# Quantum-Chemistry-Group-BNU/XTDDFT

Measured on NVIDIA B200. Metric: davidson_sigma_vectors_per_s, higher is better.
Workload: dtype f64

## Files before the change

### xtddft_b200/csrc/ozaki.cuh

```cuda
#pragma once
#include "common.cuh"

namespace xtd {

constexpr int OZ_BM = 128, OZ_BN = 64, OZ_KB = 32, OZ_STAGES = 4, OZ_MAX_S = 8, OZ_MIN_S = 3;
constexpr int OZ_THREADS = 192;
constexpr int OZ_K1_THREADS = 320;

__device__ __forceinline__ uint32_t oz_smem_u32(const void* p) { return (uint32_t)__cvta_generic_to_shared(p); }

__device__ __forceinline__ double oz_scale_of(double m) {
  if (!(m > 1e-280 && m < 1e280)) return 0.0;
  int e;
  frexp(m, &e);
  return ldexp(1.0, e - 6);
}

__global__ void oz_rowmax_t_kernel(double* __restrict__ scale, int rows_pad, const double* __restrict__ X, long ld, long sq, int rows, int K,
                                   int nq, int group, long k_valid) {
  const int row = blockIdx.x * 32 + threadIdx.x, g = blockIdx.y;
  double m = 0.0;
  if (row < rows) {
    const int q1 = min(nq, (g + 1) * group);
    for (int q = g * group; q < q1; ++q) {
      const long kmax = min((long)K, k_valid - (long)q * K);
      const double* x = X + (long)q * sq + row;
      for (long k = threadIdx.y; k < kmax; k += 32) m = fmax(m, fabs(x[k * ld]));
    }
  }
  __shared__ double red[32][33];
  red[threadIdx.y][threadIdx.x] = m;
  __syncthreads();
  if (threadIdx.y == 0) {
    for (int w = 1; w < 32; ++w) m = fmax(m, red[w][threadIdx.x]);
    if (row < rows_pad) scale[(long)g * rows_pad + row] = oz_scale_of(m);
  }
}

__global__ void oz_rowmax_kernel(double* __restrict__ scale, int rows_pad, const double* __restrict__ X, long ld, long sq, int rows, int K,
                                 int nq, int group, long k_valid) {
  const int row = blockIdx.x, g = blockIdx.y;
  double m = 0.0;
  if (row < rows) {
    const int q1 = min(nq, (g + 1) * group);
    for (int q = g * group; q < q1; ++q) {
      const int kmax = (int)min((long)K, k_valid - (long)q * K);
      const double* x = X + (long)q * sq + (long)row * ld;
      for (int k = threadIdx.x; k < kmax; k += blockDim.x) m = fmax(m, fabs(x[k]));
    }
  }
  __shared__ double red[8];
  for (int o = 16; o > 0; o >>= 1) m = fmax(m, __shfl_xor_sync(0xffffffffu, m, o));
  if ((threadIdx.x & 31) == 0) red[threadIdx.x >> 5] = m;
  __syncthreads();
  if (threadIdx.x == 0) {
    for (int w = 1; w < (int)(blockDim.x >> 5); ++w) m = fmax(m, red[w]);
    scale[(long)g * rows_pad + row] = oz_scale_of(m);
  }
}

template <int S>
__device__ __forceinline__ void oz_digits16(const double (&t)[16], uint32_t (&pk)[S][4]) {
  const double magic = 6755399441055744.0;
  if constexpr (S <= 6) {
    constexpr double SCL = (double)(1ull << (8 * (S - 1)));
    constexpr unsigned long long BAL = 128ull * (((1ull << (8 * (S - 1))) - 1ull) / 255ull);
    constexpr unsigned long long CADD = BAL - 0x4338000000000000ull;
#pragma unroll
    for (int w = 0; w < 4; ++w) {
      uint32_t lo[4], hi[4];
#pragma unroll
      for (int j = 0; j < 4; ++j) {
// ... 22 lines not shown
      for (int sl = 0; sl < S; ++sl) {
        const double u = (sl == 0) ? __dadd_rd(tt, magic) : __fma_rd(tt, 256.0, magic);
        const double qd = u - magic;
        tt = (sl == 0) ? (tt - qd) : fma(tt, 256.0, -qd);
        dg[sl] = __double2loint(u);
      }
      int carry = 0;
#pragma unroll
      for (int sl = S - 1; sl >= 1; --sl) {
        const int vv = dg[sl] + carry;
        carry = vv >= 128 ? 1 : 0;
        dg[sl] = vv - (carry << 8);
      }
      dg[0] += carry;
#pragma unroll
      for (int sl = 0; sl < S; ++sl) pk[sl][k >> 2] |= ((uint32_t)dg[sl] & 0xffu) << ((k & 3) * 8);
    }
  }
}

template <int S, bool TRANS>
__global__ void __launch_bounds__(128) oz_slice_kernel(int8_t* __restrict__ out, const double* __restrict__ scale, int rows_pad,
                                                       const double* __restrict__ X, long ld, long sq, int rows, int K, int RT, int nkb,
                                                       int group, int stacked, long k_valid) {
  const int c2 = blockIdx.x, q = blockIdx.z;
  const int row = blockIdx.y * 128 + threadIdx.x;
  const int rt = row / RT, r = row - rt * RT, nrt = rows_pad / RT;
  const int k0 = c2 * 16;
  double x[16];
#pragma unroll
  for (int k = 0; k < 16; ++k) x[k] = 0.0;
  double sc = 0.0;
  if (row < rows) {
    sc = scale[(long)(q / group) * rows_pad + row];
    const int kmax = (int)min((long)K, k_valid - (long)q * K);
    if (TRANS) {
      const double* src = X + (long)q * sq + (long)k0 * ld + row;
#pragma unroll
      for (int k = 0; k < 16; ++k)
        if (k0 + k < kmax) x[k] = src[(long)k * ld];
    } else {
      const double* src = X + (long)q * sq + (long)row * ld + k0;
      if (k0 + 16 <= kmax) {
#pragma unroll
        for (int k = 0; k < 16; k += 2) {
          const double2 v = *reinterpret_cast<const double2*>(src + k);
          x[k] = v.x;
          x[k + 1] = v.y;
        }
      } else {
#pragma unroll
        for (int k = 0; k < 16; ++k)
          if (k0 + k < kmax) x[k] = src[k];
      }
    }
  }
  const double inv = sc > 0.0 ? __hiloint2double(0x7fe00000 - __double2hiint(sc), 0) : 0.0;
  uint32_t pk[S][4];
#pragma unroll
  for (int k = 0; k < 16; ++k) x[k] *= inv;
  oz_digits16<S>(x, pk);
  int8_t* dst = out + ((((long)q * nrt + rt) * nkb + (c2 >> 1)) * S) * ((long)RT * OZ_KB) + (long)r * 16 +
                (stacked ? (long)(c2 & 1) * S * RT * 16 : (long)(c2 & 1) * RT * 16);
  const long plane = stacked ? (long)RT * 16 : (long)RT * OZ_KB;
#pragma unroll
// ... 364 lines not shown
#pragma unroll
        for (int k = 0; k < HC; ++k) acc[k] = fma(v[k], sa * sb[k], acc[k]);
      }
      double* w = p.W + zb * p.w_bstride + ((long)sp * p.Mpad + mt * OZ_BM + row) * p.Npad + nt * OZ_BN + half * HC;
#pragma unroll
      for (int c = 0; c < HC; c += 2) *reinterpret_cast<double2*>(w + c) = make_double2(p.alpha * acc[c], p.alpha * acc[c + 1]);
    }
  }
  asm volatile("tcgen05.fence::before_thread_sync;" ::: "memory");
  __syncthreads();
  if (warp == 1) {
    asm volatile("tcgen05.fence::after_thread_sync;" ::: "memory");
    asm volatile("tcgen05.dealloc.cta_group::1.sync.aligned.b32 %0, %1;" ::"r"(tmem_base), "r"(512u) : "memory");
  }
}

struct OzK1Params {
  const int8_t* A;
  const int8_t* B;
  const double* sa;
  const double* sb;
  const double* so;
  int8_t* out;
  int np, nit, nbt, nkb1, nvec, no, group, nmt2, nkb2, Mpad2;
  int it0, nit_run;
  int i_lo, i_hi;
  long ntiles;
};

template <int S>
__global__ void __launch_bounds__(OZ_K1_THREADS, 1) oz_k1_kernel(const OzK1Params p) {
  constexpr int A_SLICE = OZ_BM * OZ_KB, B_SLICE = OZ_BN * OZ_KB;
  constexpr int A_BYTES = S * A_SLICE, B_BYTES = S * B_SLICE, STAGE = A_BYTES + B_BYTES;
  extern __shared__ __align__(128) uint8_t oz_smem[];
  uint64_t* full = reinterpret_cast<uint64_t*>(oz_smem + OZ_STAGES * STAGE);
  uint64_t* empty = full + OZ_STAGES;
  uint64_t* tmem_full = empty + OZ_STAGES;
  uint64_t* tmem_empty = tmem_full + 1;
  uint32_t* tmem_slot = reinterpret_cast<uint32_t*>(tmem_empty + 1);
  const int warp = threadIdx.x >> 5, lane = threadIdx.x & 31;

  if (threadIdx.x == 0) {
    for (int s = 0; s < OZ_STAGES; ++s) {
      oz_mbar_init(&full[s], 1);
      oz_mbar_init(&empty[s], 1);
    }
    oz_mbar_init(tmem_full, 1);
    oz_mbar_init(tmem_empty, OZ_K1_THREADS - 64);
    asm volatile("fence.mbarrier_init.release.cluster;" ::: "memory");
    asm volatile("fence.proxy.async.shared::cta;" ::: "memory");
  }
  if (warp == 1) {
    asm volatile("tcgen05.alloc.cta_group::1.sync.aligned.shared::cta.b32 [%0], %1;" ::"r"(oz_smem_u32(tmem_slot)), "r"(512u) : "memory");
    asm volatile("tcgen05.relinquish_alloc_permit.cta_group::1.sync.aligned;" ::: "memory");
  }
  asm volatile("tcgen05.fence::before_thread_sync;" ::: "memory");
  __syncthreads();
  asm volatile("tcgen05.fence::after_thread_sync;" ::: "memory");
  const uint32_t tmem_base = *tmem_slot;
  const long per_p = (long)p.nit_run * p.nvec * p.nbt, per_it = (long)p.nvec * p.nbt;

  if (warp == 0) {
    if (lane == 0) {
      long it = 0;
      for (long t = blockIdx.x; t < p.ntiles; t += gridDim.x) {
        const int P = (int)(t / per_p);
        const long r0 = t - (long)P * per_p;
        const int itile = (int)(r0 / per_it);
        const long r1 = r0 - (long)itile * per_it;
        const int x = (int)(r1 / p.nbt), bt = (int)(r1 - (long)x * p.nbt);
        const int8_t* a = p.A + (((long)P * p.nit + p.it0 + itile) * p.nkb1) * A_BYTES;
        const int8_t* b = p.B + (((long)x * p.nbt + bt) * p.nkb1) * B_BYTES;
        for (int kb = 0; kb < p.nkb1; ++kb, ++it) {
          const int s = (int)(it % OZ_STAGES);
          const uint32_t ph = (uint32_t)((it / OZ_STAGES) & 1);
          oz_mbar_wait(&empty[s], ph ^ 1u);
          oz_mbar_expect_tx(&full[s], STAGE);
          uint8_t* sa = oz_smem + s * STAGE;
          oz_bulk_load(sa, a + (long)kb * A_BYTES, A_BYTES, &full[s]);
          oz_bulk_load(sa + A_BYTES, b + (long)kb * B_BYTES, B_BYTES, &full[s]);
        }
      }
    }
  } else if (warp == 1) {
    if (lane == 0) {
      constexpr uint32_t idesc0 = (2u << 4) | (1u << 7) | (1u << 10) | ((uint32_t)(OZ_BM >> 4) << 24);
      const uint32_t smem_base = oz_smem_u32(oz_smem);
      long it = 0, n = 0;
      for (long t = blockIdx.x; t < p.ntiles; t += gridDim.x, ++n) {
        if (n > 0) oz_mbar_wait(tmem_empty, (uint32_t)((n - 1) & 1));
        asm volatile("tcgen05.fence::after_thread_sync;" ::: "memory");
        for (int kb = 0; kb < p.nkb1; ++kb, ++it) {
          const int s = (int)(it % OZ_STAGES);
          const uint32_t ph = (uint32_t)((it / OZ_STAGES) & 1);
          oz_mbar_wait(&full[s], ph);
          asm volatile("tcgen05.fence::after_thread_sync;" ::: "memory");
          const uint32_t a_base = smem_base + s * STAGE, b_base = a_base + A_BYTES;
          const uint32_t later = kb > 0 ? 1u : 0u;
#pragma unroll
          for (int i = 0; i < S; ++i) {
            const uint64_t da = oz_smem_desc(a_base + i * A_SLICE, OZ_BM * 16, 128);
#pragma unroll
            for (int j0 = 0; j0 < S - i; j0 += 4) {
              const int nj = (S - i - j0) < 4 ? (S - i - j0) : 4;
              const uint64_t db = oz_smem_desc(b_base + j0 * (OZ_BN * 16), S * OZ_BN * 16, 128);
              const uint32_t idesc = idesc0 | ((uint32_t)((nj * OZ_BN) >> 3) << 17);
              oz_mma_i8(tmem_base + (uint32_t)((i + j0) * OZ_BN), da, db, idesc, (i > 0) ? 1u : later);
            }
          }
          oz_commit(&empty[s]);
        }
        oz_commit(tmem_full);
      }
    }
  } else {
    const int quad = warp & 3, half = (warp - 2) >> 2;
    const int row = quad * 32 + lane;
    const uint32_t taddr = tmem_base + ((uint32_t)(quad * 32) << 16);
    const double magic = 6755399441055744.0;
    const int rowsA = p.nit * OZ_BM, rowsB = p.nbt * OZ_BN;
    long n = 0;
    for (long t = blockIdx.x; t < p.ntiles; t += gridDim.x, ++n) {
      const int P = (int)(t / per_p);
      const long r0 = t - (long)P * per_p;
      const int itile = p.it0 + (int)(r0 / per_it);
      const long r1 = r0 - (long)(itile - p.it0) * per_it;
      const int x = (int)(r1 / p.nbt), bt = (int)(r1 - (long)x * p.nbt);
      const int i = itile * OZ_BM + row;
      const bool valid = i >= p.i_lo && i < p.i_hi;
      const int m = x * p.no + i;
      const double sa = valid ? p.sa[(long)P * rowsA + i] : 0.0;
      const double so = valid ? p.so[(long)(P / p.group) * p.Mpad2 + m] : 0.0;
      const double inv = so > 0.0 ? __hiloint2double(0x7fe00000 - __double2hiint(so), 0) : 0.0;
      const double f = sa * inv;
      const double* sb = p.sb + (long)x * rowsB + bt * OZ_BN;
      int8_t* dst = p.out + ((((long)P * p.nmt2 + (m >> 7)) * p.nkb2 + bt * 2) * S) * (long)A_SLICE + (long)(m & 127) * 16;
      oz_mbar_wait(tmem_full, (uint32_t)(n & 1));
      asm volatile("tcgen05.fence::after_thread_sync;" ::: "memory");
      constexpr int HC = OZ_BN / 2;
      double v[HC];
#pragma unroll
      for (int k = 0; k < HC; ++k) v[k] = 0.0;
#pragma unroll
      for (int l = S - 1; l >= 0; --l) {
        uint32_t r[HC];
#pragma unroll
        for (int cc = 0; cc < HC; cc += 16) oz_tmem_ld16(taddr + (uint32_t)(l * OZ_BN + half * HC + cc), r + cc);
        asm volatile("tcgen05.wait::ld.sync.aligned;" ::: "memory");
#pragma unroll
        for (int k = 0; k < HC; ++k)
          v[k] = fma(v[k], 0.00390625, __hiloint2double(0x43300000, (int)(r[k] ^ 0x80000000u)) - 4503601774854144.0);
      }
      asm volatile("tcgen05.fence::before_thread_sync;" ::: "memory");
      oz_mbar_arrive(tmem_empty);
#pragma unroll
      for (int cc = 0; cc < HC; cc += 16) {
        const int c0 = half * HC + cc;
        uint32_t pk[S][4];
        double tt[16];
#pragma unroll
        for (int k = 0; k < 16; ++k) tt[k] = v[cc + k] * (f * sb[c0 + k]);
        oz_digits16<S>(tt, pk);
        if (valid && bt * 2 + (c0 >> 5) < p.nkb2) {
          int8_t* d = dst + (long)(c0 >> 5) * S * A_SLICE + ((c0 >> 4) & 1) * (OZ_BM * 16);
#pragma unroll
          for (int sl = 0; sl < S; ++sl) *reinterpret_cast<uint4*>(d + (long)sl * A_SLICE) = make_uint4(pk[sl][0], pk[sl][1], pk[sl][2], pk[sl][3]);
        }
      }
    }
  }
  asm volatile("tcgen05.fence::before_thread_sync;" ::: "memory");
  __syncthreads();
  if (warp == 1) {
    asm volatile("tcgen05.fence::after_thread_sync;" ::: "memory");
    asm volatile("tcgen05.dealloc.cta_group::1.sync.aligned.b32 %0, %1;" ::"r"(tmem_base), "r"(512u) : "memory");
  }
}

__global__ void oz_rownorm_kernel(double* __restrict__ out, int rows_pad, const double* __restrict__ X, long ld, long sq, int rows, int K) {
  const int row = blockIdx.x, q = blockIdx.y;
  double a = 0.0;
  if (row < rows) {
    const double* x = X + (long)q * sq + (long)row * ld;
    for (int k = threadIdx.x; k < K; k += blockDim.x) a = fma(x[k], x[k], a);
  }
  __shared__ double red[8];
  for (int o = 16; o > 0; o >>= 1) a += __shfl_xor_sync(0xffffffffu, a, o);
  if ((threadIdx.x & 31) == 0) red[threadIdx.x >> 5] = a;
  __syncthreads();
  if (threadIdx.x == 0) {
    for (int w = 1; w < (int)(blockDim.x >> 5); ++w) a += red[w];
    out[(long)q * rows_pad + row] = sqrt(a);
  }
}
__global__ void oz_colmax_kernel(double* __restrict__ zmax, const double* __restrict__ norms, int rows_pad, int rows) {
// ... 7 lines not shown
  if (threadIdx.x == 0) {
    for (int w = 1; w < (int)(blockDim.x >> 5); ++w) m = fmax(m, red[w]);
    zmax[x] = m;
  }
}
__global__ void oz_bound_scale_kernel(double* __restrict__ so, int Mpad2, const double* __restrict__ loo_norm, int rowsA, const double* __restrict__ zmax,
                                      int np, int group, int nvec, int no, int i_lo, int i_hi) {
  const int m = blockIdx.x * blockDim.x + threadIdx.x, g = blockIdx.y;
  if (m >= Mpad2) return;
  double s = 0.0;
  if (m < nvec * no) {
    const int x = m / no, i = m - x * no;
    if (i < i_lo || i >= i_hi) return;
    double nl = 0.0;
    const int p1 = min(np, (g + 1) * group);
    for (int P = g * group; P < p1; ++P) nl = fmax(nl, loo_norm[(long)P * rowsA + i]);
    s = oz_scale_of(nl * zmax[x] * (1.0 + 1e-9));
  } else if (i_lo != 0) {
    return;
  }
  so[(long)g * Mpad2 + m] = s;
}

template <int S>
inline int oz_k1_launch(const OzK1Params& p, int num_sms, cudaStream_t st) {
  static bool attr_set[64] = {false};
  int dev = 0;
  XTD_CUDA(cudaGetDevice(&dev));
  if (!attr_set[dev & 63]) {
    XTD_CUDA(cudaFuncSetAttribute(oz_k1_kernel<S>, cudaFuncAttributeMaxDynamicSharedMemorySize, (int)((size_t)OZ_STAGES * S * (OZ_BM + OZ_BN) * OZ_KB + 256)));
    attr_set[dev & 63] = true;
  }
  const unsigned grid = (unsigned)std::min<long>(p.ntiles, num_sms);
  oz_k1_kernel<S><<<grid, OZ_K1_THREADS, (size_t)OZ_STAGES * S * (OZ_BM + OZ_BN) * OZ_KB + 256, st>>>(p);
  XTD_COUNT_LAUNCH();
  XTD_CUDA(cudaGetLastError());
  return XTD_OK;
}

inline int oz_k1(int S, const OzK1Params& p, int num_sms, cudaStream_t st) {
  switch (S) {
    case 3: return oz_k1_launch<3>(p, num_sms, st);
    case 4: return oz_k1_launch<4>(p, num_sms, st);
    case 5: return oz_k1_launch<5>(p, num_sms, st);
    case 6: return oz_k1_launch<6>(p, num_sms, st);
    case 7: return oz_k1_launch<7>(p, num_sms, st);
    case 8: return oz_k1_launch<8>(p, num_sms, st);
  }
  XTD_SET_ERR("oz_k1: %d slices (3..8)", S);
  return XTD_ERR_ARG;
}

struct OzShape {
  int rows = 0, RT = 0, rows_pad = 0, nrt = 0, K = 0, nkb = 0;
  void set(int rows_, int RT_, int K_) {
    rows = rows_; RT = RT_; K = K_;
    rows_pad = (int)round_up(rows_, 128);
    nrt = rows_pad / RT_;
    nkb = (int)cdiv(K_, OZ_KB);
  }
  size_t slice_bytes(long nq, int S) const { return (size_t)nq * nrt * nkb * S * RT * OZ_KB; }
  size_t scale_doubles(long nq, int group) const { return (size_t)cdiv(nq, group) * rows_pad; }
};

inline size_t oz_gemm_smem(int S) { return (size_t)OZ_STAGES * S * (OZ_BM + OZ_BN) * OZ_KB + 256; }

inline int oz_max_group(int K, int S) {
  const long kpad = round_up(K, OZ_KB);
  const long g = ((1L << 31) - 1) / ((long)S * 16384 * kpad);
  return (int)std::max<long>(g, 0);
}

template <int S>
inline int oz_slice_launch(int8_t* out, double* scale, const OzShape& sh, const double* X, long ld, long sq, int nq, int group,
                           bool trans, long k_valid, cudaStream_t st) {
  const int ng = (int)cdiv(nq, group);
  const int stacked = sh.RT == OZ_BN ? 1 : 0;
  const dim3 sgrid(2 * sh.nkb, sh.rows_pad / 128, nq);
  if (trans) {
    oz_rowmax_t_kernel<<<dim3(sh.rows_pad / 32, ng), dim3(32, 32), 0, st>>>(scale, sh.rows_pad, X, ld, sq, sh.rows, sh.K, nq, group, k_valid);
    XTD_COUNT_LAUNCH();
    XTD_CUDA(cudaGetLastError());
    oz_slice_kernel<S, true><<<sgrid, 128, 0, st>>>(out, scale, sh.rows_pad, X, ld, sq, sh.rows, sh.K, sh.RT, sh.nkb, group, stacked, k_valid);
  } else {
    oz_rowmax_kernel<<<dim3(sh.rows_pad, ng), 256, 0, st>>>(scale, sh.rows_pad, X, ld, sq, sh.rows, sh.K, nq, group, k_valid);
    XTD_COUNT_LAUNCH();
    XTD_CUDA(cudaGetLastError());
    oz_slice_kernel<S, false><<<sgrid, 128, 0, st>>>(out, scale, sh.rows_pad, X, ld, sq, sh.rows, sh.K, sh.RT, sh.nkb, group, stacked, k_valid);
  }
  XTD_COUNT_LAUNCH();
  XTD_CUDA(cudaGetLastError());
  return XTD_OK;
}

inline int oz_slice(int S, int8_t* out, double* scale, const OzShape& sh, const double* X, long ld, long sq, int nq, int group,
                    cudaStream_t st, bool trans = false, long k_valid = 0) {
  XTD_REQUIRE(nq >= 1 && nq <= 65535, XTD_ERR_ARG, "oz_slice: %d q-slices per launch (1..65535)", nq);
  XTD_REQUIRE(trans || (ld % 2 == 0 && sq % 2 == 0 && ((uintptr_t)X & 15) == 0), XTD_ERR_ALIGN,
              "oz_slice: operand must be 16-byte aligned with even strides");
  if (k_valid <= 0) k_valid = (long)nq * sh.K;
  switch (S) {
    case 3: return oz_slice_launch<3>(out, scale, sh, X, ld, sq, nq, group, trans, k_valid, st);
    case 4: return oz_slice_launch<4>(out, scale, sh, X, ld, sq, nq, group, trans, k_valid, st);
    case 5: return oz_slice_launch<5>(out, scale, sh, X, ld, sq, nq, group, trans, k_valid, st);
    case 6: return oz_slice_launch<6>(out, scale, sh, X, ld, sq, nq, group, trans, k_valid, st);
    case 7: return oz_slice_launch<7>(out, scale, sh, X, ld, sq, nq, group, trans, k_valid, st);
    case 8: return oz_slice_launch<8>(out, scale, sh, X, ld, sq, nq, group, trans, k_valid, st);
  }
  XTD_SET_ERR("oz_slice: %d slices (3..8)", S);
  return XTD_ERR_ARG;
}

template <int S, int CN>
inline int oz_gemm_launch_cn(const OzGemmParams& p, cudaStream_t st) {
  static bool attr_set[64] = {false};
  int dev = 0;
  XTD_CUDA(cudaGetDevice(&dev));
  if (!attr_set[dev & 63]) {
    XTD_CUDA(cudaFuncSetAttribute(oz_gemm_kernel<S, CN>, cudaFuncAttributeMaxDynamicSharedMemorySize, (int)oz_gemm_smem(S)));
    attr_set[dev & 63] = true;
  }
  cudaLaunchConfig_t cfg = {};
  cfg.gridDim = dim3((unsigned)(p.nmt * p.nnt * p.splits), (unsigned)p.batches);
  cfg.blockDim = dim3(OZ_THREADS);
  cfg.dynamicSmemBytes = oz_gemm_smem(S);
  cfg.stream = st;
  cudaLaunchAttribute attr[1];
  attr[0].id = cudaLaunchAttributeClusterDimension;
  attr[0].val.clusterDim.x = CN;
  attr[0].val.clusterDim.y = 1;
// ... 70 lines not shown
```

### xtddft_b200/csrc/xtd_api.cu

```cuda
#include "../../include/xtd_sigma.h"
#include "gemm.cuh"
#include "kernels.cuh"
#include "ozaki.cuh"
#include "davidson.cuh"

#include <cuda_profiler_api.h>

#include <algorithm>
#include <cstring>
#include <vector>

namespace xtd {
thread_local char g_last_error[512] = {0};
unsigned long long g_launch_count = 0;

struct DevBuf {
  double* p = nullptr;
  size_t bytes = 0;
  DevBuf() = default;
  DevBuf(const DevBuf&) = delete;
  DevBuf& operator=(const DevBuf&) = delete;
  ~DevBuf() { release(); }
  int alloc(size_t n_doubles, cudaStream_t s) {
    release();
// ... 15 lines not shown
  std::vector<std::pair<int, int>> o_blocks, v_blocks;
  long ldz, ldzt, ldco, ldcv, ldN;
  DevBuf Co, Cv, CoT, CvT;
  DevBuf Loo[2], Lvv[2];
  DevBuf Loob[2][2];
  bool need_split[2] = {false, false};
  DevBuf Lvo[2];
  bool need_narrow[2] = {false, false};
  DevBuf Lvt[2];
  DevBuf Lov[2];
  bool need_kt[2] = {false, false};
  int tail_start = 0, tail_w = 0;
  long ldoo, ldvv;
  bool need_k[2] = {false, false};
  bool use_oz[2] = {false, false};
  int8_t* LvvS[2] = {nullptr, nullptr};
  double* LvvScale[2] = {nullptr, nullptr};
  OzShape ozB;
  int oz_group = 0;
  int oz_col0[2] = {0, 0};
  int8_t* LooS[2] = {nullptr, nullptr};
  double *LooScale[2] = {nullptr, nullptr}, *LooNorm[2] = {nullptr, nullptr};
  OzShape ozL;
  bool xc_oz = false;
  int8_t *phivF = nullptr, *phivB = nullptr;
  double *phivFs = nullptr, *phivBs = nullptr;
  OzShape ozPF, ozPB;
  bool xc_oz_split = false;
  int8_t *phiF = nullptr, *phiB = nullptr;
  double *phiFs = nullptr, *phiBs = nullptr;
  OzShape ozOF, ozOB;
  DevBuf phi;
  long ldphi = 0;
  DevBuf phiv;
  long ldphiv = 0;
  long *g_indptr = nullptr, *g_cols = nullptr;
  double* g_vals = nullptr;
  long g_nnz = 0;
};

constexpr long XC_SPLIT_SMEM_MAX = 200 * 1024;
constexpr int XC_OP_MAX_NVEC = 8;
constexpr int OZ_XC_KQ = 8192;
constexpr int NARROW_MAX = 16;

struct KTermRec {
// ... 593 lines not shown
    XTD_TRY(c->Loo[tensor].alloc((size_t)naux_local * c->no * c->ldoo, h->stream));
    c->use_oz[tensor] = false;
    c->oz_col0[tensor] = 0;
    if (h->oz_slices > 0 && oz_max_group(c->nv, h->oz_slices) >= 1) {
      int n_uni = 0, n_blk = 0;
      for (const KTermRec& k : h->kterms)
        if (k.tensor == tensor && h->ch[k.ch] == c) (k.uniform ? n_uni : n_blk)++;
      if (n_blk == 0) c->use_oz[tensor] = n_uni > 0;
      else if (n_uni == 0) {
        if (c->v_blocks.size() == 1) c->use_oz[tensor] = true;
        else if (c->need_narrow[tensor]) { c->use_oz[tensor] = true; c->oz_col0[tensor] = c->v_blocks[1].first; }
      }
      if (c->use_oz[tensor]) c->tail_w = 0;
    }
    if (c->use_oz[tensor]) {
      c->ozB.set(c->nv - c->oz_col0[tensor], OZ_BN, c->nv);
      c->oz_group = std::min(4, oz_max_group(c->nv, h->oz_slices));
      if (c->LvvS[tensor]) cudaFree(c->LvvS[tensor]);
      if (c->LvvScale[tensor]) cudaFree(c->LvvScale[tensor]);
      c->LvvS[tensor] = nullptr; c->LvvScale[tensor] = nullptr;
      XTD_CUDA(cudaMalloc((void**)&c->LvvS[tensor], std::max<size_t>(c->ozB.slice_bytes(naux_local, h->oz_slices), 16)));
      XTD_CUDA(cudaMalloc((void**)&c->LvvScale[tensor], std::max<size_t>(c->ozB.scale_doubles(naux_local, c->oz_group), 2) * 8));
      c->Lvv[tensor].release();
      c->ozL.set(c->no, OZ_BM, c->no);
      if (c->LooS[tensor]) cudaFree(c->LooS[tensor]);
      if (c->LooScale[tensor]) cudaFree(c->LooScale[tensor]);
      if (c->LooNorm[tensor]) cudaFree(c->LooNorm[tensor]);
      c->LooS[tensor] = nullptr; c->LooScale[tensor] = c->LooNorm[tensor] = nullptr;
      XTD_CUDA(cudaMalloc((void**)&c->LooS[tensor], std::max<size_t>(c->ozL.slice_bytes(naux_local, h->oz_slices), 16)));
      XTD_CUDA(cudaMalloc((void**)&c->LooScale[tensor], std::max<size_t>((size_t)naux_local * c->ozL.rows_pad, 2) * 8));
      XTD_CUDA(cudaMalloc((void**)&c->LooNorm[tensor], std::max<size_t>((size_t)naux_local * c->ozL.rows_pad, 2) * 8));
    } else {
      XTD_TRY(c->Lvv[tensor].alloc((size_t)naux_local * c->nv * c->ldvv, h->stream));
    }
    if (c->need_narrow[tensor]) XTD_TRY(c->Lvo[tensor].alloc((size_t)naux_local * c->v_blocks[1].first * c->ldvv, h->stream));
    if (c->need_narrow[tensor] && c->tail_w > 0) XTD_TRY(c->Lvt[tensor].alloc((size_t)naux_local * c->tail_w * c->ldvv, h->stream));
    if (c->need_split[tensor]) {
      const int o2 = c->o_blocks[1].first;
      XTD_TRY(c->Loob[tensor][0].alloc((size_t)naux_local * o2 * c->ldoo, h->stream));
      XTD_TRY(c->Loob[tensor][1].alloc((size_t)naux_local * (c->no - o2) * c->ldoo, h->stream));
    }
  }
  if (tensor == 0)
    for (auto* j : h->jblocks) XTD_TRY(j->L.alloc((size_t)naux_local * j->nr * j->ld, h->stream));
  return XTD_OK;
}

int xtd_df_add(xtd_handle h, int tensor, const double* l_dev, long np, long ld_row, long stride_p, int packed) {
  XTD_REQUIRE(h && (tensor == 0 || tensor == 1) && l_dev && np > 0, XTD_ERR_ARG, "xtd_df_add: bad arguments");
  XTD_REQUIRE(h->naux_filled[tensor] + np <= h->naux[tensor], XTD_ERR_ARG, "xtd_df_add: more aux rows than declared (%ld + %ld > %ld)",
              h->naux_filled[tensor], np, h->naux[tensor]);
  const int N = h->nao;
  const long ldN = h->ldN;
  cudaStream_t s = h->stream;
// ... 73 lines not shown
      f.M = nmo; f.N = nmo; f.K = pn * nu_;
      f.C = h->kopen.p; f.ldc = h->ld_mo; f.accumulate = true;
      XTD_TRY(gemm(h->gemm, f, s));
    }
    for (size_t ci = 0; ci < h->ch.size(); ++ci) {
      Channel* c = h->ch[ci];
      bool need_o = c->need_k[tensor] || c->need_kt[tensor];
      if (tensor == 0)
        for (auto* j : h->jblocks) need_o = need_o || (j->ch == (int)ci);
      if (need_o) {
        GemmDesc d;
        d.A = view2d(c->CoT.p, ldN, c->no, N); d.B = Lv; d.M = c->no; d.N = N; d.K = N;
        d.batches = pn; d.z_div = 1; d.a_hi = 0; d.b_hi = 1;
        d.C = half; d.ldc = ldN; d.c_batch_stride = (long)c->no * ldN;
        XTD_TRY(gemm(h->gemm, d, s));
        MatView Hv = view3d(half, ldN, (long)c->no * ldN, pn, c->no, N);
        if (c->need_k[tensor]) {
          GemmDesc e;
          e.A = Hv; e.B = view2d(c->CoT.p, ldN, c->no, N); e.M = c->no; e.N = c->no; e.K = N;
          e.batches = pn; e.a_hi = 1; e.b_hi = 0;
          e.C = c->Loo[tensor].p + P0 * c->no * c->ldoo; e.ldc = c->ldoo; e.c_batch_stride = (long)c->no * c->ldoo;
          XTD_TRY(gemm(h->gemm, e, s));
          if (c->use_oz[tensor]) {
            const double* lc = c->Loo[tensor].p + P0 * c->no * c->ldoo;
            XTD_TRY(oz_slice(h->oz_slices, c->LooS[tensor] + c->ozL.slice_bytes(P0, h->oz_slices), c->LooScale[tensor] + (size_t)P0 * c->ozL.rows_pad,
                             c->ozL, lc, c->ldoo, (long)c->no * c->ldoo, pn, 1, s));
            oz_rownorm_kernel<<<dim3(c->ozL.rows_pad, pn), 128, 0, s>>>(c->LooNorm[tensor] + (size_t)P0 * c->ozL.rows_pad, c->ozL.rows_pad, lc, c->ldoo,
                                                                        (long)c->no * c->ldoo, c->no, c->no);
            LAUNCH_CHECK();
          }
          if (c->need_split[tensor]) {
            const int o2 = c->o_blocks[1].first;
            const int r0s[2] = {0, o2}, nrs[2] = {o2, c->no - o2};
            for (int ib = 0; ib < 2; ++ib) {
              GemmDesc f = e;
              f.A = view3d(half, ldN, (long)c->no * ldN, pn, nrs[ib], N, r0s[ib], 0);
              f.M = nrs[ib];
              f.C = c->Loob[tensor][ib].p + P0 * nrs[ib] * c->ldoo; f.c_batch_stride = (long)nrs[ib] * c->ldoo;
              XTD_TRY(gemm(h->gemm, f, s));
            }
          }
        }
        if (c->need_kt[tensor]) {
          GemmDesc e;
          e.A = Hv; e.B = view2d(c->CvT.p, ldN, c->nv, N);
          e.M = c->no; e.N = c->nv; e.K = N; e.batches = pn; e.a_hi = 1; e.b_hi = 0;
          e.C = c->Lov[tensor].p + P0 * c->no * c->ldz; e.ldc = c->ldz; e.c_batch_stride = (long)c->no * c->ldz;
          XTD_TRY(gemm(h->gemm, e, s));
        }
        if (tensor == 0)
          for (auto* j : h->jblocks) {
// ... 739 lines not shown
    PhaseTimer t(h, XTD_T_K2_SLICE);
    for (int ip = 0; ip < npass; ++ip) {
      const double* zt = h->ZT[k.ch];
      if (!k.uniform) {
        scale_blocks_kernel<<<dim3((unsigned)cdiv(ch->no, 128), ch->nv, nvec), 128, 0, s>>>(zts_tmp, h->ZT[k.ch], ch->ldzt, (long)ch->nv * ch->ldzt,
                                                                                          ch->nv, ch->no, passes[ip].bs);
        LAUNCH_CHECK();
        zt = zts_tmp;
      }
      XTD_TRY(oz_slice(S, ztS[ip], ztScale[ip], shZt, zt, ch->ldzt, (long)ch->nv * ch->ldzt, nvec, 1, s));
      oz_rownorm_kernel<<<dim3(shZt.rows_pad, nvec), 128, 0, s>>>(ztNorm, shZt.rows_pad, zt, ch->ldzt, (long)ch->nv * ch->ldzt, ch->nv, ch->no);
      LAUNCH_CHECK();
      oz_colmax_kernel<<<nvec, 256, 0, s>>>(zmax[ip], ztNorm, shZt.rows_pad, ch->nv);
      LAUNCH_CHECK();
    }
  }
  for (long P0 = 0; P0 < naux; P0 += pc) {
    const int pn = (int)std::min<long>(pc, naux - P0);
    const int ng = (int)cdiv(pn, G);
    {
      PhaseTimer t(h, XTD_T_K1);
      for (int ip = 0; ip < npass; ++ip) {
        const RowPass& rp = passes[ip];
        oz_bound_scale_kernel<<<dim3((unsigned)cdiv(shA.rows_pad, 256), ng), 256, 0, s>>>(so, shA.rows_pad, ch->LooNorm[k.tensor] + (size_t)P0 * shL.rows_pad,
                                                                                          shL.rows_pad, zmax[ip], pn, G, nvec, ch->no, rp.i_lo, rp.i_hi);
        LAUNCH_CHECK();
        OzK1Params q;
        q.A = ch->LooS[k.tensor] + shL.slice_bytes(P0, S); q.B = ztS[ip];
        q.sa = ch->LooScale[k.tensor] + (size_t)P0 * shL.rows_pad; q.sb = ztScale[ip]; q.so = so; q.out = As;
        q.np = pn; q.nit = shL.nrt; q.nbt = shZt.nrt; q.nkb1 = shL.nkb; q.nvec = nvec; q.no = ch->no; q.group = G;
        q.nmt2 = shA.nrt; q.nkb2 = shA.nkb; q.Mpad2 = shA.rows_pad;
        q.i_lo = rp.i_lo; q.i_hi = rp.i_hi;
        q.it0 = rp.i_lo / OZ_BM; q.nit_run = (rp.i_hi - 1) / OZ_BM - q.it0 + 1;
        q.ntiles = (long)pn * q.nit_run * nvec * q.nbt;
        XTD_TRY(oz_k1(S, q, h->gemm.num_sms, s));
        h->gemm.flops += 2.0 * pn * (double)(rp.i_hi - rp.i_lo) * ch->no * ch->nv * nvec;
      }
    }
    {
      PhaseTimer t(h, XTD_T_K2);
      OzGemmParams p;
      p.A = As; p.B = ch->LvvS[k.tensor]; p.sa = so; p.sb = ch->LvvScale[k.tensor];
      p.nmt = shA.nrt; p.nnt = shB.nrt; p.nkb = shA.nkb; p.nq = pn; p.group = G; p.b_q0 = (int)P0;
      p.Mpad = shA.rows_pad; p.Npad = shB.rows_pad;
      p.splits = std::min(splits_max, oz_choose_splits(tiles, ng, h->gemm.num_sms));
      p.W = W; p.alpha = k.uniform ? k.w[0][0][0][0] : 1.0;
      XTD_TRY(oz_gemm(S, p, s));
      const int M = nvec * ch->no, N = ch->nv - col0;
      const long nblk = cdiv((long)M * N, 256);
      reduce_splits_kernel<<<dim3((unsigned)(nblk > 4096 ? 4096 : nblk), 1), 256, 0, s>>>(
          h->SIG + h->sig_base[k.ch] + col0, ch->ldz, 0, W, shB.rows_pad, 0, (long)shA.rows_pad * shB.rows_pad, p.splits, M, N, 1, 0, 0, 0);
      LAUNCH_CHECK();
      h->gemm.flops += 2.0 * M * N * (double)ch->nv * pn;
    }
  }
  return XTD_OK;
}

// ... 903 lines not shown
```

Baseline: 9.482.

## Pack Loo rows across aux groups and multicast A tiles in 2-CTA clusters

Loo slices are now packed so that G auxiliary indices share one row dimension, with rows split at the occupied-block boundary. This fills the 128-row M tiles instead of padding a small `no` to 128 per P. The K1 fused kernel now runs as 2-CTA clusters where each CTA loads half of the shared A tile and multicasts it to both, while each processes a different B tile. Empty-buffer barriers count two arrivals and commits are multicast, which adds cluster synchronization and index unpacking overhead in the epilogue. Warps whose rows are all invalid skip the store path.

```diff
diff --git a/xtddft_b200/csrc/ozaki.cuh b/xtddft_b200/csrc/ozaki.cuh
--- a/xtddft_b200/csrc/ozaki.cuh
+++ b/xtddft_b200/csrc/ozaki.cuh
@@ -8,6 +8,32 @@
 constexpr int OZ_K1_THREADS = 320;
 
 __device__ __forceinline__ uint32_t oz_smem_u32(const void* p) { return (uint32_t)__cvta_generic_to_shared(p); }
+
+__host__ __device__ __forceinline__ bool oz_unpack_row(int r, int G, int o2, int no, int& P, int& i) {
+  if (r < G * o2) {
+    P = r / o2;
+    i = r - P * o2;
+    return true;
+  }
+  const int n1 = no - o2, r1 = r - G * o2;
+  if (r1 >= G * n1) return false;
+  P = r1 / n1;
+  i = o2 + (r1 - P * n1);
+  return true;
+}
+inline int oz_packed_row_lo(int i_lo, int G, int o2) { return i_lo >= o2 ? G * o2 : 0; }
+inline int oz_packed_row_hi(int i_hi, int G, int o2, int no) { return i_hi <= o2 ? G * o2 : G * no; }
+
+struct OzRowPack {
+  int G = 0, o2 = 0, no = 0, np = 0;
+  long sp = 0;
+};
+__device__ __forceinline__ long oz_src_row(const OzRowPack& pk, int q, int row, int rows, long ld) {
+  if (pk.G == 0) return row < rows ? (long)row * ld : -1L;
+  int P, i;
+  if (!oz_unpack_row(row, pk.G, pk.o2, pk.no, P, i) || q * pk.G + P >= pk.np) return -1L;
+  return (long)P * pk.sp + (long)i * ld;
+}
 
 __device__ __forceinline__ double oz_scale_of(double m) {
   if (!(m > 1e-280 && m < 1e280)) return 0.0;
@@ -38,16 +64,16 @@
 }
 
 __global__ void oz_rowmax_kernel(double* __restrict__ scale, int rows_pad, const double* __restrict__ X, long ld, long sq, int rows, int K,
-                                 int nq, int group, long k_valid) {
+                                 int nq, int group, long k_valid, const OzRowPack pack) {
   const int row = blockIdx.x, g = blockIdx.y;
   double m = 0.0;
-  if (row < rows) {
-    const int q1 = min(nq, (g + 1) * group);
-    for (int q = g * group; q < q1; ++q) {
-      const int kmax = (int)min((long)K, k_valid - (long)q * K);
-      const double* x = X + (long)q * sq + (long)row * ld;
-      for (int k = threadIdx.x; k < kmax; k += blockDim.x) m = fmax(m, fabs(x[k]));
-    }
+  const int q1 = min(nq, (g + 1) * group);
+  for (int q = g * group; q < q1; ++q) {
+    const long off = oz_src_row(pack, q, row, rows, ld);
+    if (off < 0) continue;
+    const int kmax = (int)min((long)K, k_valid - (long)q * K);
+    const double* x = X + (long)q * sq + off;
+    for (int k = threadIdx.x; k < kmax; k += blockDim.x) m = fmax(m, fabs(x[k]));
   }
   __shared__ double red[8];
   for (int o = 16; o > 0; o >>= 1) m = fmax(m, __shfl_xor_sync(0xffffffffu, m, o));
@@ -116,7 +142,7 @@
 template <int S, bool TRANS>
 __global__ void __launch_bounds__(128) oz_slice_kernel(int8_t* __restrict__ out, const double* __restrict__ scale, int rows_pad,
                                                        const double* __restrict__ X, long ld, long sq, int rows, int K, int RT, int nkb,
-                                                       int group, int stacked, long k_valid) {
+                                                       int group, int stacked, long k_valid, const OzRowPack pack) {
   const int c2 = blockIdx.x, q = blockIdx.z;
   const int row = blockIdx.y * 128 + threadIdx.x;
   const int rt = row / RT, r = row - rt * RT, nrt = rows_pad / RT;
@@ -125,7 +151,8 @@
 #pragma unroll
   for (int k = 0; k < 16; ++k) x[k] = 0.0;
   double sc = 0.0;
-  if (row < rows) {
+  const long off = TRANS ? (row < rows ? 0L : -1L) : oz_src_row(pack, q, row, rows, ld);
+  if (off >= 0) {
     sc = scale[(long)(q / group) * rows_pad + row];
     const int kmax = (int)min((long)K, k_valid - (long)q * K);
     if (TRANS) {
@@ -134,7 +161,7 @@
       for (int k = 0; k < 16; ++k)
         if (k0 + k < kmax) x[k] = src[(long)k * ld];
     } else {
-      const double* src = X + (long)q * sq + (long)row * ld + k0;
+      const double* src = X + (long)q * sq + off + k0;
       if (k0 + 16 <= kmax) {
 #pragma unroll
         for (int k = 0; k < 16; k += 2) {
@@ -545,16 +572,37 @@
   const double* sb;
   const double* so;
   int8_t* out;
-  int np, nit, nbt, nkb1, nvec, no, group, nmt2, nkb2, Mpad2;
-  int it0, nit_run;
+  int np, ntg, nbt, nkb1, nvec, no, o2, group, nmt2, nkb2, Mpad2;
+  int t0, nt_run;
   int i_lo, i_hi;
-  long ntiles;
+  long npairs;
 };
+
+struct OzK1Item {
+  int gl, tile, x, bt;
+  bool live;
+};
+__device__ __forceinline__ OzK1Item oz_k1_item(const OzK1Params& p, long u, uint32_t crank) {
+  const long nxb = (long)p.nvec * p.nbt, nxb2 = (nxb + 1) >> 1, per_g = (long)p.nt_run * nxb2;
+  OzK1Item t;
+  t.gl = (int)(u / per_g);
+  const long r0 = u - (long)t.gl * per_g;
+  const int itile = (int)(r0 / nxb2);
+  t.tile = p.t0 + itile;
+  long xb = 2 * (r0 - (long)itile * nxb2) + crank;
+  t.live = xb < nxb;
+  if (!t.live) xb = nxb - 1;
+  t.x = (int)(xb / p.nbt);
+  t.bt = (int)(xb - (long)t.x * p.nbt);
+  return t;
+}
 
 template <int S>
 __global__ void __launch_bounds__(OZ_K1_THREADS, 1) oz_k1_kernel(const OzK1Params p) {
   constexpr int A_SLICE = OZ_BM * OZ_KB, B_SLICE = OZ_BN * OZ_KB;
   constexpr int A_BYTES = S * A_SLICE, B_BYTES = S * B_SLICE, STAGE = A_BYTES + B_BYTES;
+  constexpr int A_HALF = A_BYTES / 2;
+  constexpr uint16_t cmask = 3;
   extern __shared__ __align__(128) uint8_t oz_smem[];
   uint64_t* full = reinterpret_cast<uint64_t*>(oz_smem + OZ_STAGES * STAGE);
   uint64_t* empty = full + OZ_STAGES;
@@ -562,11 +610,13 @@
   uint64_t* tmem_empty = tmem_full + 1;
   uint32_t* tmem_slot = reinterpret_cast<uint32_t*>(tmem_empty + 1);
   const int warp = threadIdx.x >> 5, lane = threadIdx.x & 31;
+  const uint32_t crank = oz_cluster_rank();
+  const long pair0 = blockIdx.x >> 1, npair_ctas = gridDim.x >> 1;
 
   if (threadIdx.x == 0) {
     for (int s = 0; s < OZ_STAGES; ++s) {
       oz_mbar_init(&full[s], 1);
-      oz_mbar_init(&empty[s], 1);
+      oz_mbar_init(&empty[s], 2);
     }
     oz_mbar_init(tmem_full, 1);
     oz_mbar_init(tmem_empty, OZ_K1_THREADS - 64);
@@ -579,28 +629,24 @@
   }
   asm volatile("tcgen05.fence::before_thread_sync;" ::: "memory");
   __syncthreads();
+  oz_cluster_sync();
   asm volatile("tcgen05.fence::after_thread_sync;" ::: "memory");
   const uint32_t tmem_base = *tmem_slot;
-  const long per_p = (long)p.nit_run * p.nvec * p.nbt, per_it = (long)p.nvec * p.nbt;
 
   if (warp == 0) {
     if (lane == 0) {
       long it = 0;
-      for (long t = blockIdx.x; t < p.ntiles; t += gridDim.x) {
-        const int P = (int)(t / per_p);
-        const long r0 = t - (long)P * per_p;
-        const int itile = (int)(r0 / per_it);
-        const long r1 = r0 - (long)itile * per_it;
-        const int x = (int)(r1 / p.nbt), bt = (int)(r1 - (long)x * p.nbt);
-        const int8_t* a = p.A + (((long)P * p.nit + p.it0 + itile) * p.nkb1) * A_BYTES;
-        const int8_t* b = p.B + (((long)x * p.nbt + bt) * p.nkb1) * B_BYTES;
+      for (long u = pair0; u < p.npairs; u += npair_ctas) {
+        const OzK1Item t = oz_k1_item(p, u, crank);
+        const int8_t* a = p.A + (((long)t.gl * p.ntg + t.tile) * p.nkb1) * A_BYTES + crank * A_HALF;
+        const int8_t* b = p.B + (((long)t.x * p.nbt + t.bt) * p.nkb1) * B_BYTES;
         for (int kb = 0; kb < p.nkb1; ++kb, ++it) {
           const int s = (int)(it % OZ_STAGES);
           const uint32_t ph = (uint32_t)((it / OZ_STAGES) & 1);
           oz_mbar_wait(&empty[s], ph ^ 1u);
           oz_mbar_expect_tx(&full[s], STAGE);
           uint8_t* sa = oz_smem + s * STAGE;
-          oz_bulk_load(sa, a + (long)kb * A_BYTES, A_BYTES, &full[s]);
+          oz_bulk_load_mc(sa + crank * A_HALF, a + (long)kb * A_BYTES, A_HALF, &full[s], cmask);
           oz_bulk_load(sa + A_BYTES, b + (long)kb * B_BYTES, B_BYTES, &full[s]);
         }
       }
@@ -610,7 +656,7 @@
       constexpr uint32_t idesc0 = (2u << 4) | (1u << 7) | (1u << 10) | ((uint32_t)(OZ_BM >> 4) << 24);
       const uint32_t smem_base = oz_smem_u32(oz_smem);
       long it = 0, n = 0;
-      for (long t = blockIdx.x; t < p.ntiles; t += gridDim.x, ++n) {
+      for (long u = pair0; u < p.npairs; u += npair_ctas, ++n) {
         if (n > 0) oz_mbar_wait(tmem_empty, (uint32_t)((n - 1) & 1));
         asm volatile("tcgen05.fence::after_thread_sync;" ::: "memory");
         for (int kb = 0; kb < p.nkb1; ++kb, ++it) {
@@ -631,7 +677,7 @@
               oz_mma_i8(tmem_base + (uint32_t)((i + j0) * OZ_BN), da, db, idesc, (i > 0) ? 1u : later);
             }
           }
-          oz_commit(&empty[s]);
+          oz_commit_mc(&empty[s], cmask);
         }
         oz_commit(tmem_full);
       }
@@ -640,20 +686,18 @@
     const int quad = warp & 3, half = (warp - 2) >> 2;
     const int row = quad * 32 + lane;
     const uint32_t taddr = tmem_base + ((uint32_t)(quad * 32) << 16);
-    const double magic = 6755399441055744.0;
-    const int rowsA = p.nit * OZ_BM, rowsB = p.nbt * OZ_BN;
+    const int rowsA = p.ntg * OZ_BM, rowsB = p.nbt * OZ_BN;
     long n = 0;
-    for (long t = blockIdx.x; t < p.ntiles; t += gridDim.x, ++n) {
-      const int P = (int)(t / per_p);
-      const long r0 = t - (long)P * per_p;
-      const int itile = p.it0 + (int)(r0 / per_it);
-      const long r1 = r0 - (long)(itile - p.it0) * per_it;
-      const int x = (int)(r1 / p.nbt), bt = (int)(r1 - (long)x * p.nbt);
-      const int i = itile * OZ_BM + row;
-      const bool valid = i >= p.i_lo && i < p.i_hi;
+    for (long u = pair0; u < p.npairs; u += npair_ctas, ++n) {
+      const OzK1Item t = oz_k1_item(p, u, crank);
+      const int x = t.x, bt = t.bt;
+      const int pr = t.tile * OZ_BM + row;
+      int Pl = 0, i = 0;
+      const bool valid = t.live && oz_unpack_row(pr, p.group, p.o2, p.no, Pl, i) && i >= p.i_lo && i < p.i_hi && t.gl * p.group + Pl < p.np;
+      const int P = t.gl * p.group + Pl;
       const int m = x * p.no + i;
-      const double sa = valid ? p.sa[(long)P * rowsA + i] : 0.0;
-      const double so = valid ? p.so[(long)(P / p.group) * p.Mpad2 + m] : 0.0;
+      const double sa = valid ? p.sa[(long)t.gl * rowsA + pr] : 0.0;
+      const double so = valid ? p.so[(long)t.gl * p.Mpad2 + m] : 0.0;
       const double inv = so > 0.0 ? __hiloint2double(0x7fe00000 - __double2hiint(so), 0) : 0.0;
       const double f = sa * inv;
       const double* sb = p.sb + (long)x * rowsB + bt * OZ_BN;
@@ -676,6 +720,7 @@
       }
       asm volatile("tcgen05.fence::before_thread_sync;" ::: "memory");
       oz_mbar_arrive(tmem_empty);
+      if (!__any_sync(0xffffffffu, valid)) continue;
 #pragma unroll
       for (int cc = 0; cc < HC; cc += 16) {
         const int c0 = half * HC + cc;
@@ -694,6 +739,7 @@
   }
   asm volatile("tcgen05.fence::before_thread_sync;" ::: "memory");
   __syncthreads();
+  oz_cluster_sync();
   if (warp == 1) {
     asm volatile("tcgen05.fence::after_thread_sync;" ::: "memory");
     asm volatile("tcgen05.dealloc.cta_group::1.sync.aligned.b32 %0, %1;" ::"r"(tmem_base), "r"(512u) : "memory");
@@ -747,30 +793,47 @@
   so[(long)g * Mpad2 + m] = s;
 }
 
+inline size_t oz_gemm_smem(int S) { return (size_t)OZ_STAGES * S * (OZ_BM + OZ_BN) * OZ_KB + 256; }
+
 template <int S>
-inline int oz_k1_launch(const OzK1Params& p, int num_sms, cudaStream_t st) {
+inline int oz_k1_launch(const OzK1Params& p, cudaStream_t st) {
   static bool attr_set[64] = {false};
+  static int max_clusters[64] = {0};
   int dev = 0;
   XTD_CUDA(cudaGetDevice(&dev));
+  cudaLaunchConfig_t cfg = {};
+  cfg.blockDim = dim3(OZ_K1_THREADS);
+  cfg.dynamicSmemBytes = oz_gemm_smem(S);
+  cfg.stream = st;
+  cudaLaunchAttribute attr[1];
+  attr[0].id = cudaLaunchAttributeClusterDimension;
+  attr[0].val.clusterDim.x = 2;
+  attr[0].val.clusterDim.y = 1;
+  attr[0].val.clusterDim.z = 1;
+  cfg.attrs = attr;
+  cfg.numAttrs = 1;
   if (!attr_set[dev & 63]) {
-    XTD_CUDA(cudaFuncSetAttribute(oz_k1_kernel<S>, cudaFuncAttributeMaxDynamicSharedMemorySize, (int)((size_t)OZ_STAGES * S * (OZ_BM + OZ_BN) * OZ_KB + 256)));
+    XTD_CUDA(cudaFuncSetAttribute(oz_k1_kernel<S>, cudaFuncAttributeMaxDynamicSharedMemorySize, (int)oz_gemm_smem(S)));
+    cfg.gridDim = dim3(2);
+    XTD_CUDA(cudaOccupancyMaxActiveClusters(&max_clusters[dev & 63], oz_k1_kernel<S>, &cfg));
+    XTD_REQUIRE(max_clusters[dev & 63] >= 1, XTD_ERR_CUDA, "oz_k1: no 2-CTA cluster of the fused half-transform fits this device");
     attr_set[dev & 63] = true;
   }
-  const unsigned grid = (unsigned)std::min<long>(p.ntiles, num_sms);
-  oz_k1_kernel<S><<<grid, OZ_K1_THREADS, (size_t)OZ_STAGES * S * (OZ_BM + OZ_BN) * OZ_KB + 256, st>>>(p);
+  cfg.gridDim = dim3((unsigned)(2 * std::min<long>(p.npairs, max_clusters[dev & 63])));
+  XTD_CUDA(cudaLaunchKernelEx(&cfg, oz_k1_kernel<S>, p));
   XTD_COUNT_LAUNCH();
   XTD_CUDA(cudaGetLastError());
   return XTD_OK;
 }
 
-inline int oz_k1(int S, const OzK1Params& p, int num_sms, cudaStream_t st) {
+inline int oz_k1(int S, const OzK1Params& p, cudaStream_t st) {
   switch (S) {
-    case 3: return oz_k1_launch<3>(p, num_sms, st);
-    case 4: return oz_k1_launch<4>(p, num_sms, st);
-    case 5: return oz_k1_launch<5>(p, num_sms, st);
-    case 6: return oz_k1_launch<6>(p, num_sms, st);
-    case 7: return oz_k1_launch<7>(p, num_sms, st);
-    case 8: return oz_k1_launch<8>(p, num_sms, st);
+    case 3: return oz_k1_launch<3>(p, st);
+    case 4: return oz_k1_launch<4>(p, st);
+    case 5: return oz_k1_launch<5>(p, st);
+    case 6: return oz_k1_launch<6>(p, st);
+    case 7: return oz_k1_launch<7>(p, st);
+    case 8: return oz_k1_launch<8>(p, st);
   }
   XTD_SET_ERR("oz_k1: %d slices (3..8)", S);
   return XTD_ERR_ARG;
@@ -788,8 +851,6 @@
   size_t scale_doubles(long nq, int group) const { return (size_t)cdiv(nq, group) * rows_pad; }
 };
 
-inline size_t oz_gemm_smem(int S) { return (size_t)OZ_STAGES * S * (OZ_BM + OZ_BN) * OZ_KB + 256; }
-
 inline int oz_max_group(int K, int S) {
   const long kpad = round_up(K, OZ_KB);
   const long g = ((1L << 31) - 1) / ((long)S * 16384 * kpad);
@@ -798,7 +859,7 @@
 
 template <int S>
 inline int oz_slice_launch(int8_t* out, double* scale, const OzShape& sh, const double* X, long ld, long sq, int nq, int group,
-                           bool trans, long k_valid, cudaStream_t st) {
+                           bool trans, long k_valid, const OzRowPack& pk, cudaStream_t st) {
   const int ng = (int)cdiv(nq, group);
   const int stacked = sh.RT == OZ_BN ? 1 : 0;
   const dim3 sgrid(2 * sh.nkb, sh.rows_pad / 128, nq);
@@ -806,12 +867,12 @@
     oz_rowmax_t_kernel<<<dim3(sh.rows_pad / 32, ng), dim3(32, 32), 0, st>>>(scale, sh.rows_pad, X, ld, sq, sh.rows, sh.K, nq, group, k_valid);
     XTD_COUNT_LAUNCH();
     XTD_CUDA(cudaGetLastError());
-    oz_slice_kernel<S, true><<<sgrid, 128, 0, st>>>(out, scale, sh.rows_pad, X, ld, sq, sh.rows, sh.K, sh.RT, sh.nkb, group, stacked, k_valid);
+    oz_slice_kernel<S, true><<<sgrid, 128, 0, st>>>(out, scale, sh.rows_pad, X, ld, sq, sh.rows, sh.K, sh.RT, sh.nkb, group, stacked, k_valid, pk);
   } else {
-    oz_rowmax_kernel<<<dim3(sh.rows_pad, ng), 256, 0, st>>>(scale, sh.rows_pad, X, ld, sq, sh.rows, sh.K, nq, group, k_valid);
+    oz_rowmax_kernel<<<dim3(sh.rows_pad, ng), 256, 0, st>>>(scale, sh.rows_pad, X, ld, sq, sh.rows, sh.K, nq, group, k_valid, pk);
     XTD_COUNT_LAUNCH();
     XTD_CUDA(cudaGetLastError());
-    oz_slice_kernel<S, false><<<sgrid, 128, 0, st>>>(out, scale, sh.rows_pad, X, ld, sq, sh.rows, sh.K, sh.RT, sh.nkb, group, stacked, k_valid);
+    oz_slice_kernel<S, false><<<sgrid, 128, 0, st>>>(out, scale, sh.rows_pad, X, ld, sq, sh.rows, sh.K, sh.RT, sh.nkb, group, stacked, k_valid, pk);
   }
   XTD_COUNT_LAUNCH();
   XTD_CUDA(cudaGetLastError());
@@ -819,18 +880,19 @@
 }
 
 inline int oz_slice(int S, int8_t* out, double* scale, const OzShape& sh, const double* X, long ld, long sq, int nq, int group,
-                    cudaStream_t st, bool trans = false, long k_valid = 0) {
+                    cudaStream_t st, bool trans = false, long k_valid = 0, const OzRowPack& pk = OzRowPack()) {
   XTD_REQUIRE(nq >= 1 && nq <= 65535, XTD_ERR_ARG, "oz_slice: %d q-slices per launch (1..65535)", nq);
-  XTD_REQUIRE(trans || (ld % 2 == 0 && sq % 2 == 0 && ((uintptr_t)X & 15) == 0), XTD_ERR_ALIGN,
+  XTD_REQUIRE(trans || (ld % 2 == 0 && sq % 2 == 0 && pk.sp % 2 == 0 && ((uintptr_t)X & 15) == 0), XTD_ERR_ALIGN,
               "oz_slice: operand must be 16-byte aligned with even strides");
+  XTD_REQUIRE(pk.G == 0 || (!trans && pk.o2 >= 1 && pk.o2 <= pk.no && pk.G * pk.no <= sh.rows_pad), XTD_ERR_ARG, "oz_slice: bad row packing");
   if (k_valid <= 0) k_valid = (long)nq * sh.K;
   switch (S) {
-    case 3: return oz_slice_launch<3>(out, scale, sh, X, ld, sq, nq, group, trans, k_valid, st);
-    case 4: return oz_slice_launch<4>(out, scale, sh, X, ld, sq, nq, group, trans, k_valid, st);
-    case 5: return oz_slice_launch<5>(out, scale, sh, X, ld, sq, nq, group, trans, k_valid, st);
-    case 6: return oz_slice_launch<6>(out, scale, sh, X, ld, sq, nq, group, trans, k_valid, st);
-    case 7: return oz_slice_launch<7>(out, scale, sh, X, ld, sq, nq, group, trans, k_valid, st);
-    case 8: return oz_slice_launch<8>(out, scale, sh, X, ld, sq, nq, group, trans, k_valid, st);
+    case 3: return oz_slice_launch<3>(out, scale, sh, X, ld, sq, nq, group, trans, k_valid, pk, st);
+    case 4: return oz_slice_launch<4>(out, scale, sh, X, ld, sq, nq, group, trans, k_valid, pk, st);
+    case 5: return oz_slice_launch<5>(out, scale, sh, X, ld, sq, nq, group, trans, k_valid, pk, st);
+    case 6: return oz_slice_launch<6>(out, scale, sh, X, ld, sq, nq, group, trans, k_valid, pk, st);
+    case 7: return oz_slice_launch<7>(out, scale, sh, X, ld, sq, nq, group, trans, k_valid, pk, st);
+    case 8: return oz_slice_launch<8>(out, scale, sh, X, ld, sq, nq, group, trans, k_valid, pk, st);
   }
   XTD_SET_ERR("oz_slice: %d slices (3..8)", S);
   return XTD_ERR_ARG;
diff --git a/xtddft_b200/csrc/xtd_api.cu b/xtddft_b200/csrc/xtd_api.cu
--- a/xtddft_b200/csrc/xtd_api.cu
+++ b/xtddft_b200/csrc/xtd_api.cu
@@ -61,6 +61,7 @@
   int8_t* LooS[2] = {nullptr, nullptr};
   double *LooScale[2] = {nullptr, nullptr}, *LooNorm[2] = {nullptr, nullptr};
   OzShape ozL;
+  int oz_row_split() const { return o_blocks.size() > 1 ? o_blocks[1].first : no; }
   bool xc_oz = false;
   int8_t *phivF = nullptr, *phivB = nullptr;
   double *phivFs = nullptr, *phivBs = nullptr;
@@ -700,14 +701,15 @@
       XTD_CUDA(cudaMalloc((void**)&c->LvvS[tensor], std::max<size_t>(c->ozB.slice_bytes(naux_local, h->oz_slices), 16)));
       XTD_CUDA(cudaMalloc((void**)&c->LvvScale[tensor], std::max<size_t>(c->ozB.scale_doubles(naux_local, c->oz_group), 2) * 8));
       c->Lvv[tensor].release();
-      c->ozL.set(c->no, OZ_BM, c->no);
+      c->ozL.set(c->oz_group * c->no, OZ_BM, c->no);
+      const long loo_groups = cdiv(naux_local, c->oz_group);
       if (c->LooS[tensor]) cudaFree(c->LooS[tensor]);
       if (c->LooScale[tensor]) cudaFree(c->LooScale[tensor]);
       if (c->LooNorm[tensor]) cudaFree(c->LooNorm[tensor]);
       c->LooS[tensor] = nullptr; c->LooScale[tensor] = c->LooNorm[tensor] = nullptr;
-      XTD_CUDA(cudaMalloc((void**)&c->LooS[tensor], std::max<size_t>(c->ozL.slice_bytes(naux_local, h->oz_slices), 16)));
-      XTD_CUDA(cudaMalloc((void**)&c->LooScale[tensor], std::max<size_t>((size_t)naux_local * c->ozL.rows_pad, 2) * 8));
-      XTD_CUDA(cudaMalloc((void**)&c->LooNorm[tensor], std::max<size_t>((size_t)naux_local * c->ozL.rows_pad, 2) * 8));
+      XTD_CUDA(cudaMalloc((void**)&c->LooS[tensor], std::max<size_t>(c->ozL.slice_bytes(loo_groups, h->oz_slices), 16)));
+      XTD_CUDA(cudaMalloc((void**)&c->LooScale[tensor], std::max<size_t>(c->ozL.scale_doubles(loo_groups, 1), 2) * 8));
+      XTD_CUDA(cudaMalloc((void**)&c->LooNorm[tensor], std::max<size_t>((size_t)naux_local * c->no, 2) * 8));
     } else {
       XTD_TRY(c->Lvv[tensor].alloc((size_t)naux_local * c->nv * c->ldvv, h->stream));
     }
@@ -827,11 +829,15 @@
           e.C = c->Loo[tensor].p + P0 * c->no * c->ldoo; e.ldc = c->ldoo; e.c_batch_stride = (long)c->no * c->ldoo;
           XTD_TRY(gemm(h->gemm, e, s));
           if (c->use_oz[tensor]) {
+            const int G = c->oz_group;
+            XTD_REQUIRE(P0 % G == 0, XTD_ERR_ARG, "xtd_df_add: aux chunk at %ld does not start a group of %d", P0, G);
             const double* lc = c->Loo[tensor].p + P0 * c->no * c->ldoo;
-            XTD_TRY(oz_slice(h->oz_slices, c->LooS[tensor] + c->ozL.slice_bytes(P0, h->oz_slices), c->LooScale[tensor] + (size_t)P0 * c->ozL.rows_pad,
-                             c->ozL, lc, c->ldoo, (long)c->no * c->ldoo, pn, 1, s));
-            oz_rownorm_kernel<<<dim3(c->ozL.rows_pad, pn), 128, 0, s>>>(c->LooNorm[tensor] + (size_t)P0 * c->ozL.rows_pad, c->ozL.rows_pad, lc, c->ldoo,
-                                                                        (long)c->no * c->ldoo, c->no, c->no);
+            OzRowPack pk;
+            pk.G = G; pk.o2 = c->oz_row_split(); pk.no = c->no; pk.np = pn; pk.sp = (long)c->no * c->ldoo;
+            XTD_TRY(oz_slice(h->oz_slices, c->LooS[tensor] + c->ozL.slice_bytes(P0 / G, h->oz_slices), c->LooScale[tensor] + (size_t)(P0 / G) * c->ozL.rows_pad,
+                             c->ozL, lc, c->ldoo, (long)G * c->no * c->ldoo, (int)cdiv(pn, G), 1, s, false, 0, pk));
+            oz_rownorm_kernel<<<dim3(c->no, pn), 128, 0, s>>>(c->LooNorm[tensor] + (size_t)P0 * c->no, c->no, lc, c->ldoo, (long)c->no * c->ldoo, c->no,
+                                                              c->no);
             LAUNCH_CHECK();
           }
           if (c->need_split[tensor]) {
@@ -1617,18 +1623,20 @@
       PhaseTimer t(h, XTD_T_K1);
       for (int ip = 0; ip < npass; ++ip) {
         const RowPass& rp = passes[ip];
-        oz_bound_scale_kernel<<<dim3((unsigned)cdiv(shA.rows_pad, 256), ng), 256, 0, s>>>(so, shA.rows_pad, ch->LooNorm[k.tensor] + (size_t)P0 * shL.rows_pad,
-                                                                                          shL.rows_pad, zmax[ip], pn, G, nvec, ch->no, rp.i_lo, rp.i_hi);
+        oz_bound_scale_kernel<<<dim3((unsigned)cdiv(shA.rows_pad, 256), ng), 256, 0, s>>>(so, shA.rows_pad, ch->LooNorm[k.tensor] + (size_t)P0 * ch->no,
+                                                                                          ch->no, zmax[ip], pn, G, nvec, ch->no, rp.i_lo, rp.i_hi);
         LAUNCH_CHECK();
+        const int o2 = ch->oz_row_split();
         OzK1Params q;
-        q.A = ch->LooS[k.tensor] + shL.slice_bytes(P0, S); q.B = ztS[ip];
-        q.sa = ch->LooScale[k.tensor] + (size_t)P0 * shL.rows_pad; q.sb = ztScale[ip]; q.so = so; q.out = As;
-        q.np = pn; q.nit = shL.nrt; q.nbt = shZt.nrt; q.nkb1 = shL.nkb; q.nvec = nvec; q.no = ch->no; q.group = G;
+        q.A = ch->LooS[k.tensor] + shL.slice_bytes(P0 / G, S); q.B = ztS[ip];
+        q.sa = ch->LooScale[k.tensor] + (size_t)(P0 / G) * shL.rows_pad; q.sb = ztScale[ip]; q.so = so; q.out = As;
+        q.np = pn; q.ntg = shL.nrt; q.nbt = shZt.nrt; q.nkb1 = shL.nkb; q.nvec = nvec; q.no = ch->no; q.o2 = o2; q.group = G;
         q.nmt2 = shA.nrt; q.nkb2 = shA.nkb; q.Mpad2 = shA.rows_pad;
         q.i_lo = rp.i_lo; q.i_hi = rp.i_hi;
-        q.it0 = rp.i_lo / OZ_BM; q.nit_run = (rp.i_hi - 1) / OZ_BM - q.it0 + 1;
-        q.ntiles = (long)pn * q.nit_run * nvec * q.nbt;
-        XTD_TRY(oz_k1(S, q, h->gemm.num_sms, s));
+        q.t0 = oz_packed_row_lo(rp.i_lo, G, o2) / OZ_BM;
+        q.nt_run = (int)cdiv(oz_packed_row_hi(rp.i_hi, G, o2, ch->no), OZ_BM) - q.t0;
+        q.npairs = (long)ng * q.nt_run * cdiv((long)nvec * q.nbt, 2);
+        XTD_TRY(oz_k1(S, q, s));
         h->gemm.flops += 2.0 * pn * (double)(rp.i_hi - rp.i_lo) * ch->no * ch->nv * nvec;
       }
     }
```

After: 9.998 (median of 6 runs). 5.4% higher.
